# Jiahao-Ma/VFA

Measured on AMD Instinct MI355X. Metric: voxels aggregated/sec (7 views->BEV grid), higher is better.
Workload: dtype f32; 1 GPU; multiviewc_200x200x1; cameras_per_rank=7, cameras_total=7, channels=256, rccl_ranks=1, parallelism=single GPU

## Files before the change

vfa_amd/csrc/vfa_fused.hip:

```cpp
#include <hip/hip_runtime.h>
#include <stdint.h>
#include <type_traits>

#include "vfa_geom.h"
#include "vfa_split.h"
#include "vfa_tile.h"

#ifndef VFA_TICKET_ORDER
#define VFA_TICKET_ORDER __ATOMIC_RELAXED
#endif

namespace {
using namespace vfa_dev;

constexpr int kRecBytes = 96;
constexpr int kMaxSlots = 123;
constexpr unsigned kItemCost = 704, kRowItemCost = 522;
constexpr int kRecSlots = 3;
constexpr int kThreads = 512;
constexpr int kRowBytes = 2 * kC;
constexpr int kPlane = kTileBoxes * kRowBytes;
constexpr int kSteps = kC / 16;

constexpr int kCont = 1 << 8;
// ... 164 lines not shown
        uint2 h0, l0, h1, l1;
        split_f16x4(src[0] * sc, src[1] * sc, src[2] * sc, src[3] * sc, h0, l0);
        split_f16x4(src[4] * sc, src[5] * sc, src[6] * sc, src[7] * sc, h1, l1);
        uh = make_uint4(h0.x, h0.y, h1.x, h1.y);
        ul = make_uint4(l0.x, l0.y, l1.x, l1.y);
    } else {
        union { __bf16 b[8]; uint4 u; } hi, lo;
#pragma unroll
        for (int k = 0; k < 8; ++k) {
            const float x = src[k];
            hi.b[k] = (__bf16)x;
            lo.b[k] = (__bf16)(x - (float)hi.b[k]);
        }
        uh = hi.u; ul = lo.u;
    }
    out[((size_t)(wave * kSteps + st) * 2 + 0) * 64 + lane] = uh;
    out[((size_t)(wave * kSteps + st) * 2 + 1) * 64 + lane] = ul;
}

struct ChunkArgs {
    const unsigned *live[kMaxScales], *overflow[kMaxScales];
    const unsigned short *item_w;
    int n_scales, n_tiles, n_views, views_pad;
    int *chunk_start, *chunk_rank;
    SplitArgs split;
    int n_split_blocks;
};
template <int G> struct TileItemsT { unsigned m[kMaxScales]; uint4 q[kMaxScales][G]; };
template <int G>
__global__ __launch_bounds__(1024) void tile_chunks_kernel(ChunkArgs a)
{
    using TileItems = TileItemsT<G>;
    constexpr bool kCache = G == 1;
    __shared__ unsigned long long part[1024];
    if (blockIdx.x > 0) {
        split_block(a.split, (int)blockIdx.x - 1, part);
        return;
    }
    const int tid = threadIdx.x, n_tiles = a.n_tiles;
    const unsigned view_mask = a.n_views >= 32 ? 0xffffffffu : ((1u << a.n_views) - 1u);
    const int per = (n_tiles + 1023) / 1024, t0 = min(n_tiles, tid * per), t1 = min(n_tiles, t0 + per);
    constexpr unsigned kScale = 294, kTile = 330, kEmpty = 32;
    struct RawTile { unsigned lv[kMaxScales], ov[kMaxScales]; uint4 q[kMaxScales][G]; };
    auto load_raw = [&](int t) {
        RawTile rt;
#pragma unroll
        for (int s = 0; s < kMaxScales; ++s) {
            const bool on = s < a.n_scales;
            const unsigned *lp = on ? a.live[s] : a.live[0], *op = on ? a.overflow[s] : a.overflow[0];
            rt.lv[s] = lp[t]; rt.ov[s] = op[t];
#pragma unroll
            for (int g = 0; g < G; ++g) {
                const int gg = g * 8 < a.n_views ? g : 0;
                rt.q[s][g] = *reinterpret_cast<const uint4 *>(a.item_w + ((size_t)t * kMaxScales + (on ? s : 0)) * a.views_pad + 8 * gg);
            }
        }
        return rt;
    };
    auto finish_tile = [&](const RawTile &rt) {
        TileItems ti;
#pragma unroll
        for (int s = 0; s < kMaxScales; ++s) {
            const bool on = s < a.n_scales;
            ti.m[s] = on ? rt.lv[s] & ~rt.ov[s] & view_mask : 0u;
#pragma unroll
            for (int g = 0; g < G; ++g) ti.q[s][g] = (!on || g * 8 >= a.n_views) ? make_uint4(0u, 0u, 0u, 0u) : rt.q[s][g];
        }
// ... 6 lines not shown
#pragma unroll
        for (int s = 0; s < kMaxScales; ++s) {
            bool first = true;
#pragma unroll
            for (int g = 0; g < G; ++g) {
                unsigned mg = (ti.m[s] >> (8 * g)) & 0xffu;
                const uint4 q = ti.q[s][g];
                const unsigned long long lo = (unsigned long long)q.x | ((unsigned long long)q.y << 32), hi = (unsigned long long)q.z | ((unsigned long long)q.w << 32);
                while (mg) {
                    const int v = __builtin_ctz(mg);
                    mg &= mg - 1u;
                    unsigned wi = (unsigned)(((v < 4 ? lo : hi) >> (16 * (v & 3))) & 0xffffull);
                    if (first) wi += kScale;
                    if (k == 0) wi += kTile;
                    first = false;
                    visit(k, w, w + wi);
                    w += wi;
                    ++k;
                }
            }
        }
        return k == 0 ? kEmpty : w;
    };
    TileItems c0 = {}, c1 = {};
    if (kCache && n_tiles > 0) {
        const RawTile r0 = load_raw(min(t0, n_tiles - 1)), r1 = load_raw(min(t0 + 1, n_tiles - 1));
        __builtin_amdgcn_sched_barrier(0);
        c0 = finish_tile(r0);
        c1 = finish_tile(r1);
    }
    auto tile_of = [&](int t) { return (kCache && t == t0) ? c0 : (kCache && t == t0 + 1) ? c1 : load_tile(t); };
    unsigned long long local = 0;
    for (int t = t0; t < t1; ++t) local += walk(tile_of(t), [](int, unsigned, unsigned) {});
    part[tid] = local;
    for (int c = tid; c <= kChunks; c += 1024) { a.chunk_start[c] = n_tiles; a.chunk_rank[c] = 0; }
    __syncthreads();
    for (int d = 1; d < 1024; d <<= 1) {
        const unsigned long long v = tid >= d ? part[tid - d] : 0ull;
        __syncthreads();
        part[tid] += v;
        __syncthreads();
    }
    const unsigned long long total = part[1023];
    unsigned long long before = part[tid] - local;
    auto pos_of = [&](long long cc) { return (total * (unsigned long long)cc + kChunks - 1) / kChunks; };
    for (int t = t0; t < t1; ++t) {
        const unsigned long long tb = before;
        long long c = tb > 0 ? (long long)((tb - 1) * kChunks / total) : 0;
        while (c < kChunks && pos_of(c) < tb) ++c;
        const TileItems ti = tile_of(t);
        int n_items = 0;
        walk(ti, [&](int kk, unsigned, unsigned) { n_items = kk + 1; });
        const unsigned w = walk(ti, [&](int kk, unsigned w0, unsigned w1) {
            while (c < kChunks) {
                const unsigned long long pc = pos_of(c);
                if (pc >= tb + w1) break;
                const int k = ((unsigned)(pc - tb) - w0) * 2 < (w1 - w0) ? kk : kk + 1;
                if (k >= n_items) { a.chunk_start[c] = t + 1 < n_tiles ? t + 1 : n_tiles; a.chunk_rank[c] = 0; }
                else { a.chunk_start[c] = t; a.chunk_rank[c] = k; }
                ++c;
            }
        });
        if (n_items == 0)
            for (; c < kChunks && pos_of(c) < tb + w; ++c) { a.chunk_start[c] = t; a.chunk_rank[c] = 0; }
        before += w;
    }
}

struct FusedScale {
    const float *integral;
    const float *bias;
    const uint4 *wfrag;
    const unsigned *live, *direct, *overflow;
    const unsigned char *hdrs, *recs;
    int Hf, Wf;
    const unsigned *amax;
    int amax_n;
};
struct FusedArgs {
    FusedScale sc[kMaxScales];
    int n_scales, n_views, L, W, tiles_w, n_tiles;
    float *out;
    const int *chunk_start, *chunk_rank;
    float *partial;
    unsigned *tickets;
    const float *rows;
    const unsigned *row_counter;
    int rows_cap;
    int accumulate;
    const int *wexp;
    int debug;
    unsigned long long *diag;
};
constexpr int kDbgNoFills = 1, kDbgNoPool = 2, kDbgNoMfma = 4, kDbgOneW = 8, kDbgNoRecords = 16, kDbgNoExtra = 32, kDbgStamps = 128;
constexpr int kDbgDumpVox = 0x1000;

struct LRec { uint4 v[6]; };

// ... 733 lines not shown
        for (int k = 0; k < 6; ++k) r[k] = rp[k];
        const float wt[16] = {__uint_as_float(r[0].x), __uint_as_float(r[0].y), __uint_as_float(r[0].z), __uint_as_float(r[0].w),
                              __uint_as_float(r[1].x), __uint_as_float(r[1].y), __uint_as_float(r[1].z), __uint_as_float(r[1].w),
                              __uint_as_float(r[2].x), __uint_as_float(r[2].y), __uint_as_float(r[2].z), __uint_as_float(r[2].w),
                              __uint_as_float(r[3].x), __uint_as_float(r[3].y), __uint_as_float(r[3].z), __uint_as_float(r[3].w)};
        const float rcp = __uint_as_float(r[4].x), masked = __uint_as_float(r[5].z), area = __uint_as_float(r[5].w);
        const bool vis = (r[4].y & (unsigned)kVis) != 0u;
        const unsigned rws[4] = {vis ? r[4].z & 0xffffu : 0u, vis ? r[4].z >> 16 : 0u, vis ? r[4].w & 0xffffu : 0u, vis ? r[4].w >> 16 : 0u};
        const unsigned cls[4] = {vis ? r[5].x & 0xffffu : 0u, vis ? r[5].x >> 16 : 0u, vis ? r[5].y & 0xffffu : 0u, vis ? r[5].y >> 16 : 0u};
        const char *img = reinterpret_cast<const char *>(a.integral) + (size_t)view * (a.Hf + 2) * Wp * kSlotBytes + q * 256 + cq * 16;
        float4 t[4][4];
#pragma unroll
        for (int i = 0; i < 4; ++i)
#pragma unroll
            for (int j = 0; j < 4; ++j) t[i][j] = *reinterpret_cast<const float4 *>(img + (size_t)(rws[i] * Wp + cls[j]) * kSlotBytes);
        __builtin_amdgcn_sched_barrier(0);
        const float4 lt = sample4(t[0][0], t[0][1], t[1][0], t[1][1], wt[0], wt[1], wt[2], wt[3]);
        const float4 rb = sample4(t[2][2], t[2][3], t[3][2], t[3][3], wt[4], wt[5], wt[6], wt[7]);
        const float4 rt = sample4(t[0][2], t[0][3], t[1][2], t[1][3], wt[8], wt[9], wt[10], wt[11]);
        const float4 lb2 = sample4(t[2][0], t[2][1], t[3][0], t[3][1], wt[12], wt[13], wt[14], wt[15]);
        float4 res = make_float4(box_mean(lt.x, rb.x, rt.x, lb2.x, area, rcp), box_mean(lt.y, rb.y, rt.y, lb2.y, area, rcp),
                                 box_mean(lt.z, rb.z, rt.z, lb2.z, area, rcp), box_mean(lt.w, rb.w, rt.w, lb2.w, area, rcp));
        if (!vis) res = make_float4(masked, masked, masked, masked);
        if (cl < a.L && cw < a.W) {
            typedef float nt4 __attribute__((ext_vector_type(4)));
            const nt4 x = {res.x, res.y, res.z, res.w};
            __builtin_nontemporal_store(x, reinterpret_cast<nt4 *>(a.vox + ((size_t)view * a.L * a.W + (size_t)cl * a.W + cw) * kC + q * 64 + cq * 4));
        }
    }
}

struct RowsArgs {
    const float *integral[kMaxScales];
    const unsigned char *recs[kMaxScales];
    int Hf[kMaxScales], Wf[kMaxScales];
    const unsigned *row_list;
    const unsigned *row_counter;
    float *rows;
    int n_tiles, rows_cap;
};
__global__ __launch_bounds__(512) void pool_rows_kernel(RowsArgs a)
{
    const int tid = threadIdx.x, wave = uniform_i(tid >> 6), lane = tid & 63, grp = lane >> 4, cq = lane & 15;
    const int count = min(uniform_i((int)*a.row_counter), a.rows_cap);
    const int b = 4 * wave + grp;
    for (int u = blockIdx.x; u < 4 * count; u += gridDim.x) {
        const int slot = u >> 2, q = u & 3;
        const unsigned e = (unsigned)uniform_i((int)a.row_list[slot]);
        const int s = (int)(e >> 30), view = (int)((e >> 25) & 31u), tile = (int)(e & 0x1ffffffu);
        const int Wp = a.Wf[s] + 2;
        const int item = view * a.n_tiles + tile;
        const uint4 *rp = reinterpret_cast<const uint4 *>(a.recs[s] + ((size_t)item * kTileBoxes + b) * kRecBytes);
        uint4 r[6];
#pragma unroll
        for (int k = 0; k < 6; ++k) r[k] = rp[k];
        const float wt[16] = {__uint_as_float(r[0].x), __uint_as_float(r[0].y), __uint_as_float(r[0].z), __uint_as_float(r[0].w),
                              __uint_as_float(r[1].x), __uint_as_float(r[1].y), __uint_as_float(r[1].z), __uint_as_float(r[1].w),
                              __uint_as_float(r[2].x), __uint_as_float(r[2].y), __uint_as_float(r[2].z), __uint_as_float(r[2].w),
                              __uint_as_float(r[3].x), __uint_as_float(r[3].y), __uint_as_float(r[3].z), __uint_as_float(r[3].w)};
        const float rcp = __uint_as_float(r[4].x), masked = __uint_as_float(r[5].z), area = __uint_as_float(r[5].w);
        const bool vis = (r[4].y & (unsigned)kVis) != 0u;
        const unsigned rws[4] = {vis ? r[4].z & 0xffffu : 0u, vis ? r[4].z >> 16 : 0u, vis ? r[4].w & 0xffffu : 0u, vis ? r[4].w >> 16 : 0u};
        const unsigned cls[4] = {vis ? r[5].x & 0xffffu : 0u, vis ? r[5].x >> 16 : 0u, vis ? r[5].y & 0xffffu : 0u, vis ? r[5].y >> 16 : 0u};
        const char *img = reinterpret_cast<const char *>(a.integral[s]) + (size_t)view * (a.Hf[s] + 2) * Wp * kSlotBytes + q * 256 + cq * 16;
        float4 t[4][4];
#pragma unroll
        for (int i = 0; i < 4; ++i)
#pragma unroll
            for (int j = 0; j < 4; ++j) t[i][j] = *reinterpret_cast<const float4 *>(img + (size_t)(rws[i] * Wp + cls[j]) * kSlotBytes);
        __builtin_amdgcn_sched_barrier(0);
        const float4 lt = sample4(t[0][0], t[0][1], t[1][0], t[1][1], wt[0], wt[1], wt[2], wt[3]);
        const float4 rb = sample4(t[2][2], t[2][3], t[3][2], t[3][3], wt[4], wt[5], wt[6], wt[7]);
        const float4 rt = sample4(t[0][2], t[0][3], t[1][2], t[1][3], wt[8], wt[9], wt[10], wt[11]);
        const float4 lb2 = sample4(t[2][0], t[2][1], t[3][0], t[3][1], wt[12], wt[13], wt[14], wt[15]);
        float4 res = make_float4(box_mean(lt.x, rb.x, rt.x, lb2.x, area, rcp), box_mean(lt.y, rb.y, rt.y, lb2.y, area, rcp),
                                 box_mean(lt.z, rb.z, rt.z, lb2.z, area, rcp), box_mean(lt.w, rb.w, rt.w, lb2.w, area, rcp));
        if (!vis) res = make_float4(masked, masked, masked, masked);
        reinterpret_cast<float4 *>(a.rows)[((size_t)slot * kTileBoxes + b) * (kC / 4) + q * 16 + cq] = res;
    }
}


struct WorkspaceLayout {
    size_t live[kMaxScales], direct[kMaxScales], overflow[kMaxScales], counter, hdrs[kMaxScales], recs[kMaxScales], wfrag[kMaxScales],
        masks_bytes, chunks, ranks, diag, rows, row_list, partial, tickets, item_w, wmax, wexp, amax, total;
    int tiles_l, tiles_w, n_tiles, rows_cap, views_pad;
};
inline WorkspaceLayout layout_of(int n_views, int L, int W, int n_scales)
{
    WorkspaceLayout w;
    w.tiles_l = (L + kTileL - 1) / kTileL;
    w.tiles_w = (W + kTileW - 1) / kTileW;
    w.n_tiles = w.tiles_l * w.tiles_w;
    size_t off = 0;
    for (int s = 0; s < kMaxScales; ++s) {
        const bool on = s < n_scales;
        w.live[s] = off;  off = align_up(off + (on ? (size_t)w.n_tiles * 4 : 0), 256);
        w.direct[s] = off; off = align_up(off + (on ? (size_t)w.n_tiles * 4 : 0), 256);
        w.overflow[s] = off; off = align_up(off + (on ? (size_t)w.n_tiles * 4 : 0), 256);
    }
    w.counter = off; off += 256;
    w.tickets = off; off = align_up(off + (size_t)w.n_tiles * sizeof(unsigned), 256);
// ... 253 lines not shown
        }
    }
    a.wexp = reinterpret_cast<const int *>(ws + lay.wexp);
    a.n_scales = n_scales; a.n_views = n_views; a.L = L; a.W = W; a.tiles_w = lay.tiles_w; a.n_tiles = lay.n_tiles;
    a.out = out; a.accumulate = accumulate;
    a.chunk_start = reinterpret_cast<const int *>(ws + lay.chunks);
    a.chunk_rank = reinterpret_cast<const int *>(ws + lay.ranks);
    a.partial = reinterpret_cast<float *>(const_cast<unsigned char *>(ws) + lay.partial);
    a.tickets = reinterpret_cast<unsigned *>(const_cast<unsigned char *>(ws) + lay.tickets);
    a.debug = debug;
    a.diag = reinterpret_cast<unsigned long long *>(const_cast<unsigned char *>(ws) + lay.diag);
    if (debug & kDbgDumpVox) {
        if (n_views != 1 || n_scales != 1 || accumulate || !out) return VFA_ERR_BAD_ARGUMENT;
        const hipError_t e = hipMemsetAsync(out, 0, (size_t)L * W * kC * sizeof(float), s);
        if (e != hipSuccess) return (int)e;
    }
    int n_cu = 256;
    {
        int dev = 0, cus = 0;
        if (hipGetDevice(&dev) == hipSuccess && hipDeviceGetAttribute(&cus, hipDeviceAttributeMultiprocessorCount, dev) == hipSuccess &&
            cus > 0)
            n_cu = cus;
    }
    if (reserved_cus > 0 && n_cu - reserved_cus >= 8) n_cu -= reserved_cus;
    int nblk = lay.n_tiles < n_cu ? lay.n_tiles : n_cu;
    nblk = (nblk + 7) / 8 * 8;
    if (nblk > kMaxBlocks) nblk = kMaxBlocks;
    a.rows = reinterpret_cast<const float *>(ws + lay.rows);
    a.row_counter = reinterpret_cast<const unsigned *>(ws + lay.counter);
    a.rows_cap = rows_cap;
    if (!(debug & 64) && !(flags & VFA_FLAG_SKIP_ROWS)) {
        RowsArgs ra;
        for (int k = 0; k < kMaxScales; ++k) {
            ra.integral[k] = a.sc[k].integral; ra.recs[k] = a.sc[k].recs;
            ra.Hf[k] = a.sc[k].Hf; ra.Wf[k] = a.sc[k].Wf;
        }
        ra.row_list = reinterpret_cast<const unsigned *>(ws + lay.row_list);
        ra.row_counter = a.row_counter;
        ra.rows = reinterpret_cast<float *>(const_cast<unsigned char *>(ws) + lay.rows);
        ra.n_tiles = lay.n_tiles; ra.rows_cap = rows_cap;
        hipLaunchKernelGGL(pool_rows_kernel, dim3(4096), dim3(512), 0, s, ra);
        const int st0 = (int)hipGetLastError();
        if (st0 || (flags & VFA_FLAG_ROWS_ONLY)) return st0;
    }
    if (debug & 64) {
        hipLaunchKernelGGL((pool_collapse_kernel<2, false, true>), dim3(nblk), dim3(kThreads), 0, s, a);
        return (int)hipGetLastError();
    }
    if (debug)
        hipLaunchKernelGGL((pool_collapse_kernel<2, true, false>), dim3(nblk), dim3(kThreads), 0, s, a);
    else if (terms == 4)
        hipLaunchKernelGGL((pool_collapse_kernel<4, false, false>), dim3(nblk), dim3(kThreads), 0, s, a);
    else if (terms == 3)
        hipLaunchKernelGGL((pool_collapse_kernel<3, false, false>), dim3(nblk), dim3(kThreads), 0, s, a);
    else
        hipLaunchKernelGGL((pool_collapse_kernel<2, false, false>), dim3(nblk), dim3(kThreads), 0, s, a);
    int st = (int)hipGetLastError();
    if (st || debug) return st;
    if ((size_t)rows_cap >= (size_t)n_views * lay.n_tiles * n_scales) return st;
    if (terms == 4)
        hipLaunchKernelGGL((pool_collapse_kernel<4, false, true>), dim3(nblk), dim3(kThreads), 0, s, a);
    else if (terms == 3)
        hipLaunchKernelGGL((pool_collapse_kernel<3, false, true>), dim3(nblk), dim3(kThreads), 0, s, a);
    else
        hipLaunchKernelGGL((pool_collapse_kernel<2, false, true>), dim3(nblk), dim3(kThreads), 0, s, a);
    return (int)hipGetLastError();
}
// ... 33 lines not shown
```

vfa_amd/csrc/vfa_tile.h:

```cpp
#ifndef VFA_TILE_H
#define VFA_TILE_H

#if defined(__HIPCC__)
#define VFA_TILE_HD __host__ __device__ __forceinline__
#else
#define VFA_TILE_HD inline
#endif

namespace vfa_dev {

constexpr int kTileW = 8, kTileL = 4, kTileBoxes = kTileW * kTileL;

struct Window { int x0, t0, b0, cwid, top_rows, bot_rows, n_slots; };

VFA_TILE_HD Window make_window(bool any_vis, int x0, int x1, int t0, int t1, int b0, int b1)
{
    Window w = {x0, t0, b0, 0, 0, 0, 0};
    if (any_vis) {
        w.cwid = x1 - x0 + 1;
        if (b0 <= t1 + 1) {
            w.top_rows = (t1 > b1 ? t1 : b1) - t0 + 1;
            w.bot_rows = 0;
            w.b0 = t0 + w.top_rows;
        } else {
            w.top_rows = t1 - t0 + 1;
            w.bot_rows = b1 - b0 + 1;
        }
        w.n_slots = w.cwid * (w.top_rows + w.bot_rows);
    }
    return w;
}
VFA_TILE_HD int slot_row(const Window &w, int y) { return y < w.t0 + w.top_rows ? y - w.t0 : w.top_rows + (y - w.b0); }
VFA_TILE_HD int window_inv(int cwid) { return cwid > 0 ? (65536 + cwid - 1) / cwid : 0; }

}

#if defined(__HIPCC__)
#include "vfa_geom.h"

namespace vfa_dev {

constexpr int kC = 256;
constexpr int kMaxScales = 3;
constexpr int kSlotBytes = kC * 4;
constexpr int kHdrBytes = 32;
constexpr int kChunks = 8192;
constexpr int kMaxBlocks = 512;
constexpr int kVis = 1;
constexpr int kTileLive = 1, kTileDirect = 2;

typedef float f32x16 __attribute__((ext_vector_type(16)));
typedef __bf16 bf16x8 __attribute__((ext_vector_type(8)));

struct ScaleDims { int Hf, Wf; };
struct Frag { bf16x8 hi, lo; };

inline size_t align_up(size_t v, size_t a) { return (v + a - 1) / a * a; }
__device__ __forceinline__ int clampi(int v, int lo, int hi) { return min(max(v, lo), hi); }

__device__ __forceinline__ float4 mul4(float4 a, float w) { return make_float4(a.x * w, a.y * w, a.z * w, a.w * w); }
__device__ __forceinline__ float4 fma4(float4 a, float w, float4 c)
{
    return make_float4(fmaf(a.x, w, c.x), fmaf(a.y, w, c.y), fmaf(a.z, w, c.z), fmaf(a.w, w, c.w));
}
__device__ __forceinline__ float4 sample4(float4 nw, float4 ne, float4 sw, float4 se, float w0, float w1, float w2, float w3)
{
// ... 85 lines not shown
```

vfa_amd/csrc/vfa_integral.hip:

```cpp
#include <hip/hip_runtime.h>
#include <stdint.h>

#include "../../include/vfa_hip.h"
#include "vfa_geom.h"
#include "vfa_split.h"

namespace {
using namespace vfa_dev;

constexpr int kMaxMaps = 4;
constexpr int kChunk = 32;

struct MapDesc {
    const float *feat;
    float *out;
    const float *scale;
    const float *shift;
    int H, W;
    unsigned row_blocks;
    unsigned long long col_vecs;
    unsigned *absmax;
};
struct MapArgs {
    MapDesc m[kMaxMaps];
    int n_maps, n_views, C;
};

template <bool AFFINE>
__global__ __launch_bounds__(kWave) void rows_batched_kernel(MapArgs a)
{
    __shared__ __align__(16) float tile[kWave][kChunk + 1];
    const int lane = threadIdx.x;
    unsigned b = blockIdx.x;
    int mi = 0;
    while (mi + 1 < a.n_maps && b >= a.m[mi].row_blocks) { b -= a.m[mi].row_blocks; ++mi; }
    const MapDesc &m = a.m[mi];
    const int H = m.H, W = m.W, C = a.C, cblocks = C / kWave;
    const int y = (int)(b % (unsigned)H);
    const unsigned rest = b / (unsigned)H;
    const int c0 = (int)(rest % (unsigned)cblocks) * kWave, v = (int)(rest / (unsigned)cblocks);
    const size_t plane = (size_t)H * W;
    const float *src = m.feat + ((size_t)v * C + c0) * plane + (size_t)y * W;
    float *dst = m.out + (((size_t)v * (H + 2) + (y + 1)) * (W + 2)) * C + c0;
// ... 108 lines not shown
    const size_t row_vecs = (size_t)(m.W + 2) * a.C / 4;
    const size_t v = i / row_vecs, r = i % row_vecs;
    float4 *p = reinterpret_cast<float4 *>(m.out) + v * (size_t)(H + 2) * row_vecs + r;
    const float4 zero = make_float4(0.f, 0.f, 0.f, 0.f);
    p[0] = zero;
    p[(size_t)(H + 1) * row_vecs] = zero;
    p += row_vecs;
    double a0 = 0.0, a1 = 0.0, a2 = 0.0, a3 = 0.0;
    auto step = [&](float4 &t) {
        a0 += (double)t.x; t.x = (float)a0;
        a1 += (double)t.y; t.y = (float)a1;
        a2 += (double)t.z; t.z = (float)a2;
        a3 += (double)t.w; t.w = (float)a3;
    };
    constexpr int U = 8;
    int y = 0;
    for (; y + U <= H; y += U) {
        float4 t[U];
#pragma unroll
        for (int k = 0; k < U; ++k) t[k] = p[(size_t)(y + k) * row_vecs];
#pragma unroll
        for (int k = 0; k < U; ++k) {
            step(t[k]);
            p[(size_t)(y + k) * row_vecs] = t[k];
        }
    }
    for (; y < H; ++y) {
        float4 t = p[(size_t)y * row_vecs];
        step(t);
        p[(size_t)y * row_vecs] = t;
    }
}

constexpr int kOpRows = 32, kOpCols = 32, kOpCh = 16, kOpThreads = kOpRows * kOpCh;
constexpr int kOpRowPitch = kOpCols * kOpCh + 16;
struct OnePassArgs {
    MapDesc m[kMaxMaps];
    unsigned unit_end[kMaxMaps];
    int split[kMaxMaps];
    int n_maps, n_views, C;
};
__device__ __forceinline__ void lds_barrier()
{
    asm volatile("s_waitcnt lgkmcnt(0)" ::: "memory");
    __builtin_amdgcn_s_barrier();
    asm volatile("" ::: "memory");
}
template <bool AFFINE>
__global__ __launch_bounds__(kOpThreads, 4) void integral_onepass_kernel(OnePassArgs a)
{
    extern __shared__ __align__(16) unsigned char op_lds[];
    float *tile = reinterpret_cast<float *>(op_lds);
    double *colacc = reinterpret_cast<double *>(op_lds + kOpRows * kOpRowPitch * 4);
    const int tid = threadIdx.x;
    unsigned u = blockIdx.x;
    int mi = 0;
    while (mi + 1 < a.n_maps && u >= a.unit_end[mi]) ++mi;
    if (mi > 0) u -= a.unit_end[mi - 1];
    const MapDesc &m = a.m[mi];
    const int H = m.H, W = m.W, C = a.C, cblocks = C / kOpCh;
    const int split = a.split[mi], part = split ? (int)(u & 1u) : 0;
    if (split) u >>= 1;
    const int v = (int)(u / (unsigned)cblocks), cb = (int)(u % (unsigned)cblocks), c0 = cb * kOpCh;
    const int r = tid >> 4, c = tid & 15;
    const size_t plane = (size_t)H * W;
    float *out_v = m.out + (size_t)v * (H + 2) * (W + 2) * C + c0;
    const int n_strips = (W + kOpCols - 1) / kOpCols;
    const int s_first = part ? split : 0, s_last = (split && !part) ? split : n_strips;
    const int xa = s_first * kOpCols, xb = min(W, s_last * kOpCols);
    {
        float *o = out_v + c;
        const int pa = part ? xa + 1 : 0, pb = (split && !part) ? xb + 1 : W + 2;
        for (int x = pa + r; x < pb; x += kOpRows) { o[(size_t)x * C] = 0.0f; o[((size_t)(H + 1) * (W + 2) + x) * C] = 0.0f; }
        for (int y = r; y < H; y += kOpRows) {
            if (!part) o[(size_t)(y + 1) * (W + 2) * C] = 0.0f;
            if (!split || part) o[((size_t)(y + 1) * (W + 2) + W + 1) * C] = 0.0f;
        }
    }
    for (int i = tid; i < (xb - xa) * kOpCh; i += kOpThreads) colacc[i] = 0.0;
    float sa = 1.0f, sb = 0.0f;
    if (AFFINE) { sa = m.scale[(size_t)v * C + c0 + c]; sb = m.shift[(size_t)v * C + c0 + c]; }
    auto act = [&](float x) {
// ... 160 lines not shown
    const size_t n = feature_stats_count(n_views, C, Hf);
    if (!integral || !absmax || max_entries <= 0 || n == 0 || n >= (1ull << 31)) return VFA_ERR_BAD_ARGUMENT;
    const unsigned grid = n < (size_t)max_entries ? (unsigned)n : (unsigned)max_entries;
    hipLaunchKernelGGL(integral_absmax_kernel, dim3(grid), dim3(kWave), 0, (hipStream_t)stream, integral, absmax, n_views, C, Hf, Wf, (unsigned)n);
    *n_entries = (int)grid;
    return (int)hipGetLastError();
}

}

extern "C" {

static int integral_images_launch(const float *const *features, const float *const *scales, const float *const *shifts,
                                  float *const *integrals, unsigned *const *absmax, int n_views, int C, int n_maps, const int *feat_hw,
                                  bool hwc, void *stream)
{
    MapArgs a = {};
    a.n_maps = n_maps; a.n_views = n_views; a.C = C;
    unsigned long long row_blocks = 0, col_vecs = 0;
    for (int s = 0; s < n_maps; ++s) {
        MapDesc &m = a.m[s];
        m.feat = features[s]; m.out = integrals[s];
        m.scale = scales ? scales[s] : nullptr; m.shift = shifts ? shifts[s] : nullptr;
        m.absmax = absmax ? absmax[s] : nullptr;
        m.H = feat_hw[2 * s]; m.W = feat_hw[2 * s + 1];
        const unsigned long long rb = (unsigned long long)m.H * (C / kWave) * n_views;
        if (rb >= (1ull << 31)) return VFA_ERR_UNSUPPORTED;
        m.row_blocks = (unsigned)rb;
        m.col_vecs = (unsigned long long)n_views * (m.W + 2) * C / 4;
        row_blocks += rb; col_vecs += m.col_vecs;
    }
    if (row_blocks >= (1ull << 31) || (col_vecs + 255) / 256 >= (1ull << 31)) return VFA_ERR_UNSUPPORTED;
    hipStream_t st = (hipStream_t)stream;
    bool onepass = !hwc && C % kOpCh == 0 && C % kWave == 0 && (long long)n_views * (C / kOpCh) >= 64;
    int w_max = 0;
    for (int s = 0; s < n_maps && onepass; ++s) {
        onepass = a.m[s].H >= 8 && a.m[s].W >= 4 && (size_t)kOpRows * kOpRowPitch * 4 + (size_t)a.m[s].W * kOpCh * 8 <= 160 * 1024 - 1024;
        w_max = a.m[s].W > w_max ? a.m[s].W : w_max;
    }
    if (onepass) {
        OnePassArgs oa = {};
        oa.n_maps = n_maps; oa.n_views = n_views; oa.C = C;
        unsigned long long units = 0;
        for (int s = 0; s < n_maps; ++s) {
            oa.m[s] = a.m[s];
            const int n_strips = (a.m[s].W + kOpCols - 1) / kOpCols;
            oa.split[s] = n_strips >= 4 ? (6 * n_strips + 5) / 10 : 0;
            units += (unsigned long long)n_views * (C / kOpCh) * (oa.split[s] ? 2 : 1);
            oa.unit_end[s] = (unsigned)units;
        }
        if (units >= (1ull << 31)) return VFA_ERR_UNSUPPORTED;
        int part_max = 0;
        for (int s = 0; s < n_maps; ++s) {
            const int left = oa.split[s] * kOpCols, wide = oa.split[s] ? (left > a.m[s].W - left ? left : a.m[s].W - left) : a.m[s].W;
            part_max = wide > part_max ? wide : part_max;
        }
        const size_t lds = (size_t)kOpRows * kOpRowPitch * 4 + (size_t)part_max * kOpCh * 8;
        auto launch = [&](auto kern) {
            hipError_t e0 = hipFuncSetAttribute(reinterpret_cast<const void *>(kern), hipFuncAttributeMaxDynamicSharedMemorySize, (int)lds);
            if (e0 != hipSuccess) return (int)e0;
            hipLaunchKernelGGL(kern, dim3((unsigned)units), dim3(kOpThreads), lds, st, oa);
            return (int)hipGetLastError();
        };
        return scales ? launch(integral_onepass_kernel<true>) : launch(integral_onepass_kernel<false>);
    }
    if (hwc) {
        if (scales) hipLaunchKernelGGL((rows_hwc_kernel<true>), dim3((unsigned)row_blocks), dim3(kWave), 0, st, a);
        else hipLaunchKernelGGL((rows_hwc_kernel<false>), dim3((unsigned)row_blocks), dim3(kWave), 0, st, a);
    } else {
        if (scales) hipLaunchKernelGGL((rows_batched_kernel<true>), dim3((unsigned)row_blocks), dim3(kWave), 0, st, a);
        else hipLaunchKernelGGL((rows_batched_kernel<false>), dim3((unsigned)row_blocks), dim3(kWave), 0, st, a);
    }
    int e = (int)hipGetLastError();
    if (e) return e;
    hipLaunchKernelGGL(cols_batched_kernel, dim3((unsigned)((col_vecs + 255) / 256)), dim3(256), 0, st, a, col_vecs);
    return (int)hipGetLastError();
}

size_t vfa_feature_stats_count(int n_views, int C, int Hf) { return vfa_dev::feature_stats_count(n_views, C, Hf); }

int vfa_integral_absmax_f32(const float *integral, unsigned *absmax, int n_views, int C, int Hf, int Wf, void *stream)
{
    if (!integral || !absmax || n_views < 0 || C <= 0 || Hf <= 0 || Wf <= 0) return VFA_ERR_BAD_ARGUMENT;
    const size_t n = vfa_feature_stats_count(n_views, C, Hf);
    if (n == 0) return 0;
    if (n >= (1ull << 31)) return VFA_ERR_UNSUPPORTED;
    hipLaunchKernelGGL(integral_absmax_kernel, dim3((unsigned)n), dim3(kWave), 0, (hipStream_t)stream, integral, absmax, n_views, C, Hf, Wf,
                       (unsigned)n);
    return (int)hipGetLastError();
}

int vfa_integral_images_f32(const float *const *features, const float *const *scales, const float *const *shifts,
                            float *const *integrals, unsigned *const *absmax, int n_views, int C, int n_maps, const int *feat_hw,
                            void *stream)
{
    if (!features || !integrals || !feat_hw || n_views < 0 || C <= 0 || n_maps < 0) return VFA_ERR_BAD_ARGUMENT;
    if ((scales == nullptr) != (shifts == nullptr)) return VFA_ERR_BAD_ARGUMENT;
// ... 43 lines not shown
```

Measured before the change: 1.519 billion voxels/s.

## Stage row-pooling integral windows in LDS and use wave-level chunk scan

The chunk planner swaps its 1024-entry shared-memory Hillis-Steele scan, which needed many block barriers, for a wave shuffle scan plus a 16-entry per-wave reduction. It also computes the starting chunk once per thread, counts items with popcount, and has only the last tile-owning wave write the tail chunk entries. pool_rows_kernel now reads each tile's header window and stages the window's integral-image slots into LDS with global_load_lds, so the 16 per-box taps come from shared memory instead of scattered global loads. This adds block-wide barriers per row item and depends on the header inverse-width encoding round-tripping correctly.

New measurement: 1.518 billion voxels/s. About the same (-0.0%).

```diff
diff --git a/vfa_amd/csrc/vfa_fused.hip b/vfa_amd/csrc/vfa_fused.hip
--- a/vfa_amd/csrc/vfa_fused.hip
+++ b/vfa_amd/csrc/vfa_fused.hip
@@ -220,7 +220,7 @@
 {
     using TileItems = TileItemsT<G>;
     constexpr bool kCache = G == 1;
-    __shared__ unsigned long long part[1024];
+    __shared__ unsigned long long part[16];
     if (blockIdx.x > 0) {
         split_block(a.split, (int)blockIdx.x - 1, part);
         return;
@@ -293,25 +293,35 @@
     auto tile_of = [&](int t) { return (kCache && t == t0) ? c0 : (kCache && t == t0 + 1) ? c1 : load_tile(t); };
     unsigned long long local = 0;
     for (int t = t0; t < t1; ++t) local += walk(tile_of(t), [](int, unsigned, unsigned) {});
-    part[tid] = local;
-    for (int c = tid; c <= kChunks; c += 1024) { a.chunk_start[c] = n_tiles; a.chunk_rank[c] = 0; }
+    const int lane = tid & 63, wave = tid >> 6;
+    unsigned long long incl = local;
+#pragma unroll
+    for (int d = 1; d < 64; d <<= 1) {
+        const unsigned long long v = __shfl_up(incl, d);
+        if (lane >= d) incl += v;
+    }
+    if (lane == 63) part[wave] = incl;
     __syncthreads();
-    for (int d = 1; d < 1024; d <<= 1) {
-        const unsigned long long v = tid >= d ? part[tid - d] : 0ull;
-        __syncthreads();
-        part[tid] += v;
-        __syncthreads();
-    }
-    const unsigned long long total = part[1023];
-    unsigned long long before = part[tid] - local;
-    auto pos_of = [&](long long cc) { return (total * (unsigned long long)cc + kChunks - 1) / kChunks; };
+    unsigned long long total = 0, waves_before = 0;
+#pragma unroll
+    for (int i = 0; i < 16; ++i) {
+        const unsigned long long v = part[i];
+        if (i < wave) waves_before += v;
+        total += v;
+    }
+    unsigned long long before = waves_before + incl - local;
+    auto pos_of = [&](int cc) { return (total * (unsigned long long)cc + kChunks - 1) / kChunks; };
+    int c = kChunks;
+    if (t0 < t1) {
+        c = before > 0 ? (int)((before - 1) * kChunks / total) : 0;
+        while (c < kChunks && pos_of(c) < before) ++c;
+    }
     for (int t = t0; t < t1; ++t) {
         const unsigned long long tb = before;
-        long long c = tb > 0 ? (long long)((tb - 1) * kChunks / total) : 0;
-        while (c < kChunks && pos_of(c) < tb) ++c;
         const TileItems ti = tile_of(t);
         int n_items = 0;
-        walk(ti, [&](int kk, unsigned, unsigned) { n_items = kk + 1; });
+#pragma unroll
+        for (int s = 0; s < kMaxScales; ++s) n_items += __builtin_popcount(ti.m[s]);
         const unsigned w = walk(ti, [&](int kk, unsigned w0, unsigned w1) {
             while (c < kChunks) {
                 const unsigned long long pc = pos_of(c);
@@ -325,6 +335,10 @@
         if (n_items == 0)
             for (; c < kChunks && pos_of(c) < tb + w; ++c) { a.chunk_start[c] = t; a.chunk_rank[c] = 0; }
         before += w;
+    }
+    const int last = (n_tiles - 1) / per;
+    if (wave == (last >> 6)) {
+        for (int cc = __shfl(c, last & 63) + lane; cc <= kChunks; cc += 64) { a.chunk_start[cc] = n_tiles; a.chunk_rank[cc] = 0; }
     }
 }
 
@@ -1124,7 +1138,7 @@
 
 struct RowsArgs {
     const float *integral[kMaxScales];
-    const unsigned char *recs[kMaxScales];
+    const unsigned char *hdrs[kMaxScales], *recs[kMaxScales];
     int Hf[kMaxScales], Wf[kMaxScales];
     const unsigned *row_list;
     const unsigned *row_counter;
@@ -1133,6 +1147,7 @@
 };
 __global__ __launch_bounds__(512) void pool_rows_kernel(RowsArgs a)
 {
+    __shared__ float4 s_win[kRowWinSlots * 16];
     const int tid = threadIdx.x, wave = uniform_i(tid >> 6), lane = tid & 63, grp = lane >> 4, cq = lane & 15;
     const int count = min(uniform_i((int)*a.row_counter), a.rows_cap);
     const int b = 4 * wave + grp;
@@ -1142,10 +1157,23 @@
         const int s = (int)(e >> 30), view = (int)((e >> 25) & 31u), tile = (int)(e & 0x1ffffffu);
         const int Wp = a.Wf[s] + 2;
         const int item = view * a.n_tiles + tile;
+        const i32x8 hd = *reinterpret_cast<const __attribute__((address_space(4))) i32x8 *>((size_t)(a.hdrs[s] + (size_t)item * kHdrBytes));
         const uint4 *rp = reinterpret_cast<const uint4 *>(a.recs[s] + ((size_t)item * kTileBoxes + b) * kRecBytes);
         uint4 r[6];
 #pragma unroll
         for (int k = 0; k < 6; ++k) r[k] = rp[k];
+        const char *img = reinterpret_cast<const char *>(a.integral[s]) + (size_t)view * (a.Hf[s] + 2) * Wp * kSlotBytes + q * 256 + cq * 16;
+        const Window win = header_window(hd[1], hd[3], hd[4], hd[5], hd[6], hd[7]);
+        const bool in_lds = win.n_slots > 0 && win.n_slots <= kRowWinSlots;
+        if (in_lds) {
+            for (int sl = 4 * wave; sl < win.n_slots; sl += 32) {
+                const int sg = min(sl + grp, win.n_slots - 1);
+                const int wr = (sg * hd[3]) >> 16, wc = sg - wr * win.cwid;
+                const int y = wr < win.top_rows ? win.t0 + wr : win.b0 + (wr - win.top_rows), x = win.x0 + wc;
+                __builtin_amdgcn_global_load_lds((const __attribute__((address_space(1))) void *)(img + ((size_t)(y + 1) * Wp + (x + 1)) * kSlotBytes),
+                                                 (__attribute__((address_space(3))) void *)(s_win + sl * 16), 16, 0, 0);
+            }
+        }
         const float wt[16] = {__uint_as_float(r[0].x), __uint_as_float(r[0].y), __uint_as_float(r[0].z), __uint_as_float(r[0].w),
                               __uint_as_float(r[1].x), __uint_as_float(r[1].y), __uint_as_float(r[1].z), __uint_as_float(r[1].w),
                               __uint_as_float(r[2].x), __uint_as_float(r[2].y), __uint_as_float(r[2].z), __uint_as_float(r[2].w),
@@ -1154,12 +1182,26 @@
         const bool vis = (r[4].y & (unsigned)kVis) != 0u;
         const unsigned rws[4] = {vis ? r[4].z & 0xffffu : 0u, vis ? r[4].z >> 16 : 0u, vis ? r[4].w & 0xffffu : 0u, vis ? r[4].w >> 16 : 0u};
         const unsigned cls[4] = {vis ? r[5].x & 0xffffu : 0u, vis ? r[5].x >> 16 : 0u, vis ? r[5].y & 0xffffu : 0u, vis ? r[5].y >> 16 : 0u};
-        const char *img = reinterpret_cast<const char *>(a.integral[s]) + (size_t)view * (a.Hf[s] + 2) * Wp * kSlotBytes + q * 256 + cq * 16;
         float4 t[4][4];
-#pragma unroll
-        for (int i = 0; i < 4; ++i)
-#pragma unroll
-            for (int j = 0; j < 4; ++j) t[i][j] = *reinterpret_cast<const float4 *>(img + (size_t)(rws[i] * Wp + cls[j]) * kSlotBytes);
+        if (in_lds) {
+            int off[4][4];
+#pragma unroll
+            for (int i = 0; i < 4; ++i)
+#pragma unroll
+                for (int j = 0; j < 4; ++j) off[i][j] = vis ? padded_slot(win, (int)rws[i], (int)cls[j]) * 16 + cq : cq;
+            __builtin_amdgcn_s_waitcnt(0x0f70);
+            __syncthreads();
+#pragma unroll
+            for (int i = 0; i < 4; ++i)
+#pragma unroll
+                for (int j = 0; j < 4; ++j) t[i][j] = s_win[off[i][j]];
+            __syncthreads();
+        } else {
+#pragma unroll
+            for (int i = 0; i < 4; ++i)
+#pragma unroll
+                for (int j = 0; j < 4; ++j) t[i][j] = *reinterpret_cast<const float4 *>(img + (size_t)(rws[i] * Wp + cls[j]) * kSlotBytes);
+        }
         __builtin_amdgcn_sched_barrier(0);
         const float4 lt = sample4(t[0][0], t[0][1], t[1][0], t[1][1], wt[0], wt[1], wt[2], wt[3]);
         const float4 rb = sample4(t[2][2], t[2][3], t[3][2], t[3][3], wt[4], wt[5], wt[6], wt[7]);
@@ -1479,7 +1521,7 @@
     if (!(debug & 64) && !(flags & VFA_FLAG_SKIP_ROWS)) {
         RowsArgs ra;
         for (int k = 0; k < kMaxScales; ++k) {
-            ra.integral[k] = a.sc[k].integral; ra.recs[k] = a.sc[k].recs;
+            ra.integral[k] = a.sc[k].integral; ra.hdrs[k] = a.sc[k].hdrs; ra.recs[k] = a.sc[k].recs;
             ra.Hf[k] = a.sc[k].Hf; ra.Wf[k] = a.sc[k].Wf;
         }
         ra.row_list = reinterpret_cast<const unsigned *>(ws + lay.row_list);
diff --git a/vfa_amd/csrc/vfa_tile.h b/vfa_amd/csrc/vfa_tile.h
--- a/vfa_amd/csrc/vfa_tile.h
+++ b/vfa_amd/csrc/vfa_tile.h
@@ -32,6 +32,16 @@
 }
 VFA_TILE_HD int slot_row(const Window &w, int y) { return y < w.t0 + w.top_rows ? y - w.t0 : w.top_rows + (y - w.b0); }
 VFA_TILE_HD int window_inv(int cwid) { return cwid > 0 ? (65536 + cwid - 1) / cwid : 0; }
+
+constexpr int kRowWinSlots = 256;
+VFA_TILE_HD int window_cwid(int inv) { return inv > 0 ? (65536 + inv - 1) / inv : 0; }
+VFA_TILE_HD Window header_window(int n_slots, int inv, int x0, int t0, int top_rows, int b0)
+{
+    Window w = {x0, t0, b0, window_cwid(inv), top_rows, 0, n_slots};
+    w.bot_rows = w.cwid > 0 ? n_slots / w.cwid - top_rows : 0;
+    return w;
+}
+VFA_TILE_HD int padded_slot(const Window &w, int py, int px) { return slot_row(w, py - 1) * w.cwid + (px - 1 - w.x0); }
 
 }
 
```

## Add two-team pipelined one-pass integral kernel with double-buffered LDS tiles

Applied to the files above, without the earlier changes.

Adds a pipelined one-pass integral-image kernel that launches twice the threads and splits them into two teams. One team loads and row-scans the next strip into one LDS tile while the other column-scans and stores the previous tile from a second buffer. Planning logic moves into a new header that picks the pipelined form when two tiles plus the column accumulator fit in the LDS budget, and otherwise falls back to the existing single-buffer kernel. The goal is to overlap global loads and row scans with column scans and stores. The cost is doubled LDS use, which lowers occupancy, plus extra barriers per strip.

Result: slower. 1.439 billion voxels/s before, 1.419 billion voxels/s after (-1.4%).

```diff
diff --git a/vfa_amd/csrc/vfa_integral.hip b/vfa_amd/csrc/vfa_integral.hip
--- a/vfa_amd/csrc/vfa_integral.hip
+++ b/vfa_amd/csrc/vfa_integral.hip
@@ -3,12 +3,13 @@
 
 #include "../../include/vfa_hip.h"
 #include "vfa_geom.h"
+#include "vfa_integral_plan.h"
 #include "vfa_split.h"
 
 namespace {
 using namespace vfa_dev;
-
-constexpr int kMaxMaps = 4;
+using namespace vfa_plan;
+
 constexpr int kChunk = 32;
 
 struct MapDesc {
@@ -183,8 +184,7 @@
     }
 }
 
-constexpr int kOpRows = 32, kOpCols = 32, kOpCh = 16, kOpThreads = kOpRows * kOpCh;
-constexpr int kOpRowPitch = kOpCols * kOpCh + 16;
+constexpr int kOpThreads = kOpRows * kOpCh;
 struct OnePassArgs {
     MapDesc m[kMaxMaps];
     unsigned unit_end[kMaxMaps];
@@ -198,7 +198,188 @@
     asm volatile("" ::: "memory");
 }
 template <bool AFFINE>
-__global__ __launch_bounds__(kOpThreads, 4) void integral_onepass_kernel(OnePassArgs a)
+__global__ __launch_bounds__(2 * kOpThreads) void integral_onepass_kernel(OnePassArgs a)
+{
+    extern __shared__ __align__(16) unsigned char op_lds[];
+    float *tiles = reinterpret_cast<float *>(op_lds);
+    double *colacc = reinterpret_cast<double *>(op_lds + 2 * kOpTileBytes);
+    constexpr int kTileFloats = kOpRows * kOpRowPitch;
+    const int tid = threadIdx.x;
+    const bool team_p = tid < kOpThreads;
+    const int t = tid & (kOpThreads - 1);
+    unsigned u = blockIdx.x;
+    int mi = 0;
+    while (mi + 1 < a.n_maps && u >= a.unit_end[mi]) ++mi;
+    if (mi > 0) u -= a.unit_end[mi - 1];
+    const MapDesc &m = a.m[mi];
+    const int H = m.H, W = m.W, C = a.C, cblocks = C / kOpCh;
+    const int split = a.split[mi], part = split ? (int)(u & 1u) : 0;
+    if (split) u >>= 1;
+    const int v = (int)(u / (unsigned)cblocks), cb = (int)(u % (unsigned)cblocks), c0 = cb * kOpCh;
+    const int r = t >> 4, c = t & 15;
+    const size_t plane = (size_t)H * W;
+    float *out_v = m.out + (size_t)v * (H + 2) * (W + 2) * C + c0;
+    const int n_strips = (W + kOpCols - 1) / kOpCols;
+    const int s_first = part ? split : 0, s_last = (split && !part) ? split : n_strips;
+    const int xa = s_first * kOpCols, xb = min(W, s_last * kOpCols);
+    {
+        float *o = out_v + c;
+        const int rb = tid >> 4;
+        const int pa = part ? xa + 1 : 0, pb = (split && !part) ? xb + 1 : W + 2;
+        for (int x = pa + rb; x < pb; x += 2 * kOpRows) { o[(size_t)x * C] = 0.0f; o[((size_t)(H + 1) * (W + 2) + x) * C] = 0.0f; }
+        for (int y = rb; y < H; y += 2 * kOpRows) {
+            if (!part) o[(size_t)(y + 1) * (W + 2) * C] = 0.0f;
+            if (!split || part) o[((size_t)(y + 1) * (W + 2) + W + 1) * C] = 0.0f;
+        }
+    }
+    for (int i = tid; i < (xb - xa) * kOpCh; i += 2 * kOpThreads) colacc[i] = 0.0;
+    float sa = 1.0f, sb = 0.0f;
+    if (AFFINE && team_p) { sa = m.scale[(size_t)v * C + c0 + c]; sb = m.shift[(size_t)v * C + c0 + c]; }
+    auto act = [&](float x) {
+        if (!AFFINE) return x;
+        float f = x * sa;
+        f = f + sb;
+        return (f < 0.0f) ? 0.0f : f;
+    };
+    unsigned amax = 0u;
+    auto load_strip = [&](float4 (&buf)[kOpCols / 4], int y0, int x0) {
+        const int x4 = t & 7;
+#pragma unroll
+        for (int j = 0; j < kOpCols / 4; ++j) {
+            const int line = (t & ~63) + 8 * j + ((t & 63) >> 3), row = line >> 4, ch = line & 15;
+            buf[j] = *reinterpret_cast<const float4 *>(m.feat + ((size_t)v * C + c0 + ch) * plane + (size_t)min(y0 + row, H - 1) * W +
+                                                       min(x0 + 4 * x4, W - 4));
+        }
+    };
+    auto col_scan = [&](float *tile, int x0, int rows, int nx) {
+        if (r < nx) {
+            double acc = colacc[(x0 - xa + r) * kOpCh + c];
+            float *tcol = tile + r * kOpCh + c;
+            if (rows == kOpRows) {
+#pragma unroll
+                for (int k = 0; k < kOpRows; ++k) {
+                    acc += (double)tcol[k * kOpRowPitch];
+                    tcol[k * kOpRowPitch] = (float)acc;
+                }
+            } else {
+                for (int k = 0; k < rows; ++k) {
+                    acc += (double)tcol[k * kOpRowPitch];
+                    tcol[k * kOpRowPitch] = (float)acc;
+                }
+            }
+            colacc[(x0 - xa + r) * kOpCh + c] = acc;
+        }
+    };
+    auto store_tile = [&](const float *tile, int y0, int x0, int rows, int nx) {
+#pragma unroll
+#ifdef VFA_INT_P_STORES
+        for (int j = 0; j < kOpCols / 8; ++j) {
+            const int idx = tid + 2 * kOpThreads * j, row = min(idx >> 7, rows - 1), x = min((idx >> 2) & 31, nx - 1), c4 = idx & 3;
+#else
+        for (int j = 0; j < kOpCols / 4; ++j) {
+            const int idx = t + kOpThreads * j, row = min(idx >> 7, rows - 1), x = min((idx >> 2) & 31, nx - 1), c4 = idx & 3;
+#endif
+            *reinterpret_cast<float4 *>(out_v + ((size_t)(y0 + row + 1) * (W + 2) + (x0 + x + 1)) * C + 4 * c4) =
+                *reinterpret_cast<const float4 *>(tile + row * kOpRowPitch + x * kOpCh + 4 * c4);
+        }
+    };
+#ifdef VFA_INT_P_STORES
+    constexpr bool kPStores = true;
+#else
+    constexpr bool kPStores = false;
+#endif
+    float4 cur[kOpCols / 4];
+    if (team_p) load_strip(cur, 0, 0);
+    int b = 0;
+    bool q_has = false;
+    int q_y0 = 0, q_x0 = 0, q_rows = 0, q_nx = 0;
+    for (int y0 = 0; y0 < H; y0 += kOpRows) {
+        const int rows = min(kOpRows, H - y0);
+        double racc = 0.0;
+        for (int s = 0; s < s_last; ++s) {
+            const int x0 = s * kOpCols, nx = min(kOpCols, W - x0);
+            const bool carry_only = s < s_first;
+            const bool last_strip = s + 1 == s_last;
+            const bool more = !last_strip || y0 + kOpRows < H;
+            float *tile_p = tiles + b * kTileFloats, *tile_q = tiles + (b ^ 1) * kTileFloats;
+            if (team_p) {
+                {
+                    float *raw = tile_p;
+#pragma unroll
+                    for (int j = 0; j < kOpCols / 4; ++j) {
+                        float *p = raw + ((t & ~63) + 8 * j + ((t & 63) >> 3)) * 33 + 4 * (t & 7);
+                        p[0] = cur[j].x; p[1] = cur[j].y; p[2] = cur[j].z; p[3] = cur[j].w;
+                    }
+#pragma unroll
+                    for (int j = 0; j < kOpCols / 4; ++j)
+                        cur[j] = make_float4(raw[t * 33 + 4 * j], raw[t * 33 + 4 * j + 1], raw[t * 33 + 4 * j + 2], raw[t * 33 + 4 * j + 3]);
+                }
+                auto raw_of = [&](int k) {
+                    const float4 q = cur[k / 4];
+                    return (k & 3) == 0 ? q.x : (k & 3) == 1 ? q.y : (k & 3) == 2 ? q.z : q.w;
+                };
+                float *trow = tile_p + r * kOpRowPitch + c;
+                if (r < rows) {
+                    if (carry_only) {
+#pragma unroll
+                        for (int k = 0; k < kOpCols; ++k) racc += (double)act(raw_of(k));
+                    } else if (nx == kOpCols) {
+#pragma unroll
+                        for (int k = 0; k < kOpCols; ++k) {
+                            const float f = act(raw_of(k));
+                            amax = max(amax, __float_as_uint(f) & 0x7fffffffu);
+                            racc += (double)f;
+                            trow[k * kOpCh] = (float)racc;
+                        }
+                    } else {
+#pragma unroll
+                        for (int k = 0; k < kOpCols; ++k) {
+                            if (k < nx) {
+                                const float f = act(raw_of(k));
+                                amax = max(amax, __float_as_uint(f) & 0x7fffffffu);
+                                racc += (double)f;
+                                trow[k * kOpCh] = (float)racc;
+                            }
+                        }
+                    }
+                }
+                if (more) load_strip(cur, last_strip ? y0 + kOpRows : y0, last_strip ? 0 : x0 + kOpCols);
+            } else if (q_has) {
+                col_scan(tile_q, q_x0, q_rows, q_nx);
+            }
+            if (q_has) {
+                lds_barrier();
+                if (kPStores || !team_p) store_tile(tile_q, q_y0, q_x0, q_rows, q_nx);
+            }
+            if (q_has || !carry_only) lds_barrier();
+            q_has = !carry_only;
+            if (q_has) { q_y0 = y0; q_x0 = x0; q_rows = rows; q_nx = nx; b ^= 1; }
+        }
+    }
+    if (q_has) {
+        float *tile_q = tiles + (b ^ 1) * kTileFloats;
+        if (!team_p) col_scan(tile_q, q_x0, q_rows, q_nx);
+        lds_barrier();
+        if (kPStores || !team_p) store_tile(tile_q, q_y0, q_x0, q_rows, q_nx);
+    }
+    if (m.absmax) {
+        __shared__ unsigned s_max[kOpThreads / kWave];
+        amax = wave_max_u32(amax);
+        if (team_p && (tid & 63) == 0) s_max[tid >> 6] = amax;
+        __syncthreads();
+        if (tid == 0) {
+            unsigned mx = 0u;
+            for (int k = 0; k < kOpThreads / kWave; ++k) mx = max(mx, s_max[k]);
+            unsigned *e = m.absmax + ((size_t)v * (C / kWave) + (cb >> 2)) * H;
+            const int q = 2 * (cb & 3) + part;
+            for (int y = q; y < H; y += 8) e[y] = y == q ? mx : 0u;
+            if (!split) for (int y = q + 1; y < H; y += 8) e[y] = 0u;
+        }
+    }
+}
+
+template <bool AFFINE>
+__global__ __launch_bounds__(kOpThreads, 4) void integral_onepass_single_kernel(OnePassArgs a)
 {
     extern __shared__ __align__(16) unsigned char op_lds[];
     float *tile = reinterpret_cast<float *>(op_lds);
@@ -425,37 +606,21 @@
     }
     if (row_blocks >= (1ull << 31) || (col_vecs + 255) / 256 >= (1ull << 31)) return VFA_ERR_UNSUPPORTED;
     hipStream_t st = (hipStream_t)stream;
-    bool onepass = !hwc && C % kOpCh == 0 && C % kWave == 0 && (long long)n_views * (C / kOpCh) >= 64;
-    int w_max = 0;
-    for (int s = 0; s < n_maps && onepass; ++s) {
-        onepass = a.m[s].H >= 8 && a.m[s].W >= 4 && (size_t)kOpRows * kOpRowPitch * 4 + (size_t)a.m[s].W * kOpCh * 8 <= 160 * 1024 - 1024;
-        w_max = a.m[s].W > w_max ? a.m[s].W : w_max;
-    }
-    if (onepass) {
+    const vfa_plan::IntegralPlan plan = vfa_plan::integral_plan(n_views, C, n_maps, feat_hw, hwc);
+    if (plan.form != vfa_plan::kTwoPass) {
+        if (plan.units >= (1ull << 31)) return VFA_ERR_UNSUPPORTED;
         OnePassArgs oa = {};
         oa.n_maps = n_maps; oa.n_views = n_views; oa.C = C;
-        unsigned long long units = 0;
-        for (int s = 0; s < n_maps; ++s) {
-            oa.m[s] = a.m[s];
-            const int n_strips = (a.m[s].W + kOpCols - 1) / kOpCols;
-            oa.split[s] = n_strips >= 4 ? (6 * n_strips + 5) / 10 : 0;
-            units += (unsigned long long)n_views * (C / kOpCh) * (oa.split[s] ? 2 : 1);
-            oa.unit_end[s] = (unsigned)units;
-        }
-        if (units >= (1ull << 31)) return VFA_ERR_UNSUPPORTED;
-        int part_max = 0;
-        for (int s = 0; s < n_maps; ++s) {
-            const int left = oa.split[s] * kOpCols, wide = oa.split[s] ? (left > a.m[s].W - left ? left : a.m[s].W - left) : a.m[s].W;
-            part_max = wide > part_max ? wide : part_max;
-        }
-        const size_t lds = (size_t)kOpRows * kOpRowPitch * 4 + (size_t)part_max * kOpCh * 8;
+        for (int s = 0; s < n_maps; ++s) { oa.m[s] = a.m[s]; oa.split[s] = plan.split[s]; oa.unit_end[s] = plan.unit_end[s]; }
+        const bool pipe = plan.form == vfa_plan::kOnePassPipe;
         auto launch = [&](auto kern) {
-            hipError_t e0 = hipFuncSetAttribute(reinterpret_cast<const void *>(kern), hipFuncAttributeMaxDynamicSharedMemorySize, (int)lds);
+            hipError_t e0 = hipFuncSetAttribute(reinterpret_cast<const void *>(kern), hipFuncAttributeMaxDynamicSharedMemorySize, (int)plan.lds);
             if (e0 != hipSuccess) return (int)e0;
-            hipLaunchKernelGGL(kern, dim3((unsigned)units), dim3(kOpThreads), lds, st, oa);
+            hipLaunchKernelGGL(kern, dim3((unsigned)plan.units), dim3(pipe ? 2 * kOpThreads : kOpThreads), plan.lds, st, oa);
             return (int)hipGetLastError();
         };
-        return scales ? launch(integral_onepass_kernel<true>) : launch(integral_onepass_kernel<false>);
+        if (pipe) return scales ? launch(integral_onepass_kernel<true>) : launch(integral_onepass_kernel<false>);
+        return scales ? launch(integral_onepass_single_kernel<true>) : launch(integral_onepass_single_kernel<false>);
     }
     if (hwc) {
         if (scales) hipLaunchKernelGGL((rows_hwc_kernel<true>), dim3((unsigned)row_blocks), dim3(kWave), 0, st, a);
diff --git a/vfa_amd/csrc/vfa_integral_plan.h b/vfa_amd/csrc/vfa_integral_plan.h
--- /dev/null
+++ b/vfa_amd/csrc/vfa_integral_plan.h
@@ -0,0 +1,51 @@
+#pragma once
+#include <stddef.h>
+
+#ifndef VFA_INT_SPLIT_MIN
+#define VFA_INT_SPLIT_MIN 4
+#endif
+namespace vfa_plan {
+
+constexpr int kMaxMaps = 4;
+constexpr int kOpRows = 32, kOpCols = 32, kOpCh = 16;
+constexpr int kOpRowPitch = kOpCols * kOpCh + 16;
+constexpr size_t kOpTileBytes = (size_t)kOpRows * kOpRowPitch * 4;
+constexpr size_t kOpLdsBudget = 160 * 1024 - 1024;
+
+enum IntegralForm {
+    kTwoPass = 0,
+    kOnePassSingle = 1,
+    kOnePassPipe = 2,
+};
+
+struct IntegralPlan {
+    int form;
+    size_t lds;
+    int split[kMaxMaps];
+    unsigned unit_end[kMaxMaps];
+    unsigned long long units;
+    int part_max;
+};
+
+inline IntegralPlan integral_plan(int n_views, int C, int n_maps, const int *feat_hw, bool hwc)
+{
+    IntegralPlan p = {};
+    bool onepass = !hwc && C % kOpCh == 0 && C % 64 == 0 && (long long)n_views * (C / kOpCh) >= 64;
+    for (int s = 0; s < n_maps && onepass; ++s)
+        onepass = feat_hw[2 * s] >= 8 && feat_hw[2 * s + 1] >= 4 && kOpTileBytes + (size_t)feat_hw[2 * s + 1] * kOpCh * 8 <= kOpLdsBudget;
+    if (!onepass) return p;
+    for (int s = 0; s < n_maps; ++s) {
+        const int W = feat_hw[2 * s + 1], n_strips = (W + kOpCols - 1) / kOpCols;
+        p.split[s] = n_strips >= VFA_INT_SPLIT_MIN ? (6 * n_strips + 5) / 10 : 0;
+        p.units += (unsigned long long)n_views * (C / kOpCh) * (p.split[s] ? 2 : 1);
+        p.unit_end[s] = (unsigned)p.units;
+        const int left = p.split[s] * kOpCols, wide = p.split[s] ? (left > W - left ? left : W - left) : W;
+        p.part_max = wide > p.part_max ? wide : p.part_max;
+    }
+    const size_t colacc = (size_t)p.part_max * kOpCh * 8;
+    p.form = 2 * kOpTileBytes + colacc <= kOpLdsBudget ? kOnePassPipe : kOnePassSingle;
+    p.lds = (p.form == kOnePassPipe ? 2 : 1) * kOpTileBytes + colacc;
+    return p;
+}
+
+}
```
